# NICTA/revrand

Measured on AMD Instinct MI355X. Metric: feature-rows/sec (Phi + PhiT Phi + PhiT y) at N=10M D=32 F=4096, higher is better.
Workload: dtype f32; 1 GPU; RandomRBF nbases=2048 (F=4096), D=32, N=10000000 f32, features + MFMA Gram, rows sharded over 1 GPU(s); rows_per_gpu=10000000, device=(gfx950:sramecc+:xnack-), gram_engine=f32

## Files before the change

### revrand_amd/csrc/rr_rff.hip

```cpp
#include "rr_syrk_args.h"
#include <algorithm>
#include <map>
#include <mutex>
#include <type_traits>




__device__ __forceinline__ void sincos_rev(float t, float &s, float &c) {
    const float f = t - __builtin_rintf(t);
    s = __builtin_amdgcn_sinf(f);
    c = __builtin_amdgcn_cosf(f);
}

__device__ __forceinline__ void sincos_rev(double t, double &s, double &c) { rr_sincos_rev_f64(t, s, c); }
typedef double doublex4 __attribute__((ext_vector_type(4)));

template <int DMAX, bool GUARD, typename TX, typename TC>
__device__ __forceinline__ TC project_row(const TX *__restrict__ xr, int d, const TC (&w)[DMAX]) {
    TC z = 0;
#pragma unroll
    for (int i = 0; i < DMAX; ++i) {
        if (!GUARD || i < d) z = fma((TC)xr[i], w[i], z);
    }
// ... 829 lines not shown
#undef RR_PAIRR

__global__ void __launch_bounds__(GR_THREADS, 2)
rr_syrk_f32_ragged_kernel(const SyrkArgs p) {
    __shared__ float lds[2 * GR_KB * GR_LD];
    const int lane = threadIdx.x & 63;
    const int wave = __builtin_amdgcn_readfirstlane(threadIdx.x >> 6);
    const int last = p.nb - 1;
    const int ta = blockIdx.x % last;
    const int ks = blockIdx.x / last;
    const int ca = last * GR_TC;
    const int cb = ta * GR_TC;
    const int64_t row_begin = (int64_t)ks * p.rows_per_split;
    int64_t row_end = row_begin + p.rows_per_split;
    if (row_end > p.rows) row_end = p.rows;
    const int64_t nkb = (row_end - row_begin) / GR_KB;
    RR_DEV_ASSERT(p.rows % GR_KB == 0 && p.rows_per_split % GR_KB == 0 && p.nb * GR_TC == p.ldp && p.F > ca);
    const int w = p.F + (p.bcol ? 1 : 0) - ca;
    int ni = (w - (wave >> 2) * 128 + 31) / 32;
    ni = ni < 0 ? 0 : (ni > 4 ? 4 : ni);
    switch (ni) {
        case 0: syrk_ragged_loop<0>(p, lds, wave, lane, ca, cb, row_begin, nkb, ks); break;
        case 1: syrk_ragged_loop<1>(p, lds, wave, lane, ca, cb, row_begin, nkb, ks); break;
        case 2: syrk_ragged_loop<2>(p, lds, wave, lane, ca, cb, row_begin, nkb, ks); break;
        case 3: syrk_ragged_loop<3>(p, lds, wave, lane, ca, cb, row_begin, nkb, ks); break;
        default: syrk_ragged_loop<4>(p, lds, wave, lane, ca, cb, row_begin, nkb, ks); break;
    }
}

__constant__ unsigned char RR_DIAG_I[8][5] = {{0, 0, 0, 0, 0}, {1, 1, 1, 1, 1}, {2, 2, 2, 2, 2}, {3, 3, 3, 3, 3},
                                              {0, 0, 0, 7, 0}, {1, 1, 6, 6, 1}, {2, 5, 5, 5, 2}, {4, 4, 4, 4, 4}};
__constant__ unsigned char RR_DIAG_J[8][5] = {{0, 1, 2, 3, 4}, {1, 2, 3, 4, 5}, {2, 3, 4, 5, 6}, {3, 4, 5, 6, 7},
                                              {5, 6, 7, 7, 5}, {6, 7, 6, 7, 6}, {7, 5, 6, 7, 7}, {4, 5, 6, 7, 4}};

template <int NB>
struct KOpsD {
    float2v a[NB], b[NB];
    template <int P>
    __device__ __forceinline__ void load(const unsigned (&abase)[NB], const unsigned (&bbase)[NB]) {
#pragma unroll
        for (int e = 0; e < NB; ++e) a[e] = lds_read2st64<16 * P, 16 * P + 8>(abase[e]);
#pragma unroll
        for (int e = 0; e < NB; ++e) b[e] = lds_read2st64<16 * P, 16 * P + 8>(bbase[e]);
    }
};

template <int NB, int FIRST, int LAST>
__device__ __forceinline__ void gram_mfma_d(const KOpsD<NB> &o, floatx16 (&acc)[NB]) {
#pragma unroll
    for (int q = FIRST; q < LAST; ++q)
        acc[q % NB] = __builtin_amdgcn_mfma_f32_32x32x2f32(o.a[q % NB][q / NB], o.b[q % NB][q / NB], acc[q % NB], 0, 0, 0);
}

#define RR_PAIRD(P, CUR, NXT)                                  \
    lds_wait();                                                \
    __builtin_amdgcn_sched_barrier(0);                         \
    gram_mfma_d<NB, 0, 1>(CUR, acc);                           \
    __builtin_amdgcn_sched_barrier(0);                         \
    if ((P) + 1 < 8) NXT.template load<((P) + 1) & 7>(abase, bbase); \
    __builtin_amdgcn_sched_barrier(0);                         \
    gram_mfma_d<NB, 1, 2 * NB>(CUR, acc);                      \
    __builtin_amdgcn_sched_barrier(0);

template <int NB>
__device__ __forceinline__ void syrk_diag_body(const SyrkArgs &p, float *lds, int wave, int lane) {
    const int ta = blockIdx.x % p.nb;
    const int ks = blockIdx.x / p.nb;
    const int ca = ta * GR_TC;

    const int64_t row_begin = (int64_t)ks * p.rows_per_split;
    int64_t row_end = row_begin + p.rows_per_split;
    if (row_end > p.rows) row_end = p.rows;

    const unsigned lds0 = (unsigned)(size_t)(__attribute__((address_space(3))) float *)lds;
    const unsigned lane_off = 4u * ((lane >> 5) * GR_TC + (lane & 31));
    int bi[NB], bj[NB];
#pragma unroll
    for (int e = 0; e < NB; ++e) {
        bi[e] = RR_DIAG_I[wave][e];
        bj[e] = RR_DIAG_J[wave][e];
    }
    floatx16 acc[NB];
#pragma unroll
    for (int e = 0; e < NB; ++e)
#pragma unroll
        for (int k = 0; k < 16; ++k) acc[e][k] = 0.f;

    auto dma_tile = [&](float *buf, int64_t kb0) {
#pragma unroll
        for (int k = 0; k < 4; ++k) {
            const int lr = 4 * wave + k;
            RR_DEV_ASSERT(kb0 + lr < p.rows && ca + GR_TC <= p.ldp && p.rows % GR_KB == 0 && p.rows_per_split % GR_KB == 0);
            const float *src = p.P + (kb0 + lr) * p.ldp + ca + 4 * lane;
            __builtin_amdgcn_global_load_lds((gptr_t)src, (lptr_t)(buf + lr * GR_TC), 16, 0, 0);
        }
    };

    const int64_t nkb = (row_end - row_begin) / GR_KB;
    if (nkb > 0) {
        dma_tile(lds, row_begin);
        __syncthreads();
        for (int64_t kb = 0; kb < nkb; ++kb) {
            const int cbuf = (int)(kb & 1);
            if (kb + 1 < nkb) dma_tile(lds + (cbuf ^ 1) * (GR_KB * GR_TC), row_begin + (kb + 1) * GR_KB);
            unsigned abase[NB], bbase[NB];
#pragma unroll
            for (int e = 0; e < NB; ++e) {
                abase[e] = lds0 + cbuf * (4u * GR_KB * GR_TC) + lane_off + 128u * bi[e];
                bbase[e] = lds0 + cbuf * (4u * GR_KB * GR_TC) + lane_off + 128u * bj[e];
            }
            KOpsD<NB> o0, o1;
            o0.template load<0>(abase, bbase);
            RR_PAIRD(0, o0, o1) RR_PAIRD(1, o1, o0) RR_PAIRD(2, o0, o1) RR_PAIRD(3, o1, o0)
            RR_PAIRD(4, o0, o1) RR_PAIRD(5, o1, o0) RR_PAIRD(6, o0, o1) RR_PAIRD(7, o1, o0)
            __syncthreads();
        }
    }

    const int64_t F = p.F;
    const int hi = lane >> 5;
#pragma unroll
    for (int e = 0; e < NB; ++e) {
        const int64_t gc = ca + 32 * bj[e] + (lane & 31);
#pragma unroll
        for (int k = 0; k < 16; ++k) {
            const int64_t gr = ca + 32 * bi[e] + (k & 3) + 8 * (k >> 2) + 4 * hi;
            if (gr <= gc) rr_syrk_out(p, ks, gr, gc, acc[e][k]);
        }
    }
    (void)F;
}
#undef RR_PAIRD

__global__ void __launch_bounds__(GR_THREADS, 2)
rr_syrk_f32_diag_kernel(const SyrkArgs p) {
    __shared__ float lds[2 * GR_KB * GR_TC];
    const int lane = threadIdx.x & 63;
    const int wave = __builtin_amdgcn_readfirstlane(threadIdx.x >> 6);
    if (wave < 4)
        syrk_diag_body<5>(p, lds, wave, lane);
    else
        syrk_diag_body<4>(p, lds, wave, lane);
}

typedef float floatx4 __attribute__((ext_vector_type(4)));

template <int OFF>
__device__ __forceinline__ float lds_read_b32_off(unsigned addr) {
    float r;
    asm volatile("ds_read_b32 %0, %1 offset:%2" : "=v"(r) : "v"(addr), "i"(OFF));
    return r;
}

template <int NB, int ED>
struct KOpsD16 {
    float2v a[NB], b[NB];
    float x0, x1;
    template <int P>
    __device__ __forceinline__ void load(const unsigned (&abase)[NB], const unsigned (&bbase)[NB], unsigned xbase) {
#pragma unroll
        for (int e = 0; e < NB; ++e)
            if (e != ED) a[e] = lds_read2st64<16 * P, 16 * P + 8>(abase[e]);
#pragma unroll
        for (int e = 0; e < NB; ++e)
            if (e != ED) b[e] = lds_read2st64<16 * P, 16 * P + 8>(bbase[e]);
        x0 = lds_read_b32_off<4096 * P>(xbase);
        x1 = lds_read_b32_off<4096 * P + 64>(xbase);
    }
};

template <int NB, int ED, int FIRST, int LAST>
__device__ __forceinline__ void gram_mfma_d16(const KOpsD16<NB, ED> &o, floatx16 (&acc)[NB], floatx4 (&dd)[3]) {
#pragma unroll
    for (int q = FIRST; q < LAST; ++q) {
        if (q < NB - 1 || q >= NB + 2) {
            const int s_ = q < NB - 1 ? 0 : 1;
            const int r_ = q < NB - 1 ? q : q - (NB + 2);
            const int e = r_ < ED ? r_ : r_ + 1;
            acc[e] = __builtin_amdgcn_mfma_f32_32x32x2f32(o.a[e][s_], o.b[e][s_], acc[e], 0, 0, 0);
        } else {
            const int t = q - (NB - 1);
            dd[t] = __builtin_amdgcn_mfma_f32_16x16x4f32(t == 2 ? o.x1 : o.x0, t == 0 ? o.x0 : o.x1, dd[t], 0, 0, 0);
        }
    }
}

#define RR_PAIRD16(P, CUR, NXT)                                \
    lds_wait();                                                \
    __builtin_amdgcn_sched_barrier(0);                         \
    gram_mfma_d16<NB, ED, 0, 1>(CUR, acc, dd);                 \
    __builtin_amdgcn_sched_barrier(0);                         \
    if ((P) + 1 < KB / 4) NXT.template load<((P) + 1) & (KB / 4 - 1)>(abase, bbase, xbase); \
    __builtin_amdgcn_sched_barrier(0);                         \
    gram_mfma_d16<NB, ED, 1, 2 * NB + 1>(CUR, acc, dd);        \
    __builtin_amdgcn_sched_barrier(0);

template <int NB, int ED, int KB>
__device__ __forceinline__ void syrk_diag16_body(const SyrkArgs &p, float *lds, int wave, int lane, const unsigned bid) {
    const int ta = bid % p.nb;
    const int ks = bid / p.nb;
    const int ca = ta * GR_TC;
    const int64_t row_begin = (int64_t)ks * p.rows_per_split;
    int64_t row_end = row_begin + p.rows_per_split;
    if (row_end > p.rows) row_end = p.rows;

    const unsigned lds0 = (unsigned)(size_t)(__attribute__((address_space(3))) float *)lds;
    const unsigned lane_off = 4u * ((lane >> 5) * GR_TC + (lane & 31));
    int bi[NB], bj[NB];
#pragma unroll
    for (int e = 0; e < NB; ++e) {
        bi[e] = RR_DIAG_I[wave][e];
        bj[e] = RR_DIAG_J[wave][e];
    }
    RR_DEV_ASSERT(bi[ED] == bj[ED]);
    const unsigned lane_off16 = 4u * ((lane >> 4) * GR_TC + 32 * bi[ED] + (lane & 15));
    floatx16 acc[NB];
    floatx4 dd[3];
#pragma unroll
    for (int e = 0; e < NB; ++e)
#pragma unroll
        for (int k = 0; k < 16; ++k) acc[e][k] = 0.f;
#pragma unroll
    for (int t = 0; t < 3; ++t) dd[t] = floatx4{0.f, 0.f, 0.f, 0.f};

    const unsigned voff = 16u * lane, ldp4 = (unsigned)p.ldp * 4u;
    auto dma_tile = [&](float *buf, int64_t kb0) {
        RR_DEV_ASSERT(kb0 + KB <= p.rows && ca + GR_TC <= p.ldp && p.rows % KB == 0 && p.rows_per_split % KB == 0);
        const rr_rsrc_t ra = rr_make_rsrc(p.P + kb0 * p.ldp + ca, 0x7fffffffu);
#pragma unroll
        for (int k = 0; k < KB / 8; ++k) {
            const int lr = (KB / 8) * wave + k;
            __builtin_amdgcn_raw_ptr_buffer_load_lds(ra, (lptr_t)(buf + lr * GR_TC), 16, voff, (unsigned)lr * ldp4, 0, 0);
        }
    };

    const int64_t nkb = (row_end - row_begin) / KB;
    if (nkb > 0) {
        dma_tile(lds, row_begin);
        __syncthreads();
        for (int64_t kb = 0; kb < nkb; ++kb) {
            const int cbuf = (int)(kb & 1);
            const int slot = p.spread ? rr_dma_slot(wave, p.spread) : 0;
            auto dma_next = [&]() {
                if (kb + 1 < nkb) dma_tile(lds + (cbuf ^ 1) * (KB * GR_TC), row_begin + (kb + 1) * KB);
            };
            if (slot == 0) dma_next();
            unsigned abase[NB], bbase[NB];
#pragma unroll
            for (int e = 0; e < NB; ++e) {
                abase[e] = lds0 + cbuf * (4u * KB * GR_TC) + lane_off + 128u * bi[e];
                bbase[e] = lds0 + cbuf * (4u * KB * GR_TC) + lane_off + 128u * bj[e];
            }
            const unsigned xbase = lds0 + cbuf * (4u * KB * GR_TC) + lane_off16;
            KOpsD16<NB, ED> o0, o1;
            o0.template load<0>(abase, bbase, xbase);
            RR_PAIRD16(0, o0, o1)
            if (slot == 1) dma_next();
            RR_PAIRD16(1, o1, o0)
            if (slot == 2) dma_next();
            RR_PAIRD16(2, o0, o1)
            if (slot == 3) dma_next();
            RR_PAIRD16(3, o1, o0)
            RR_PAIRD16(4, o0, o1) RR_PAIRD16(5, o1, o0) RR_PAIRD16(6, o0, o1) RR_PAIRD16(7, o1, o0)
            if constexpr (KB == 64) {
                RR_PAIRD16(8, o0, o1) RR_PAIRD16(9, o1, o0) RR_PAIRD16(10, o0, o1) RR_PAIRD16(11, o1, o0)
                RR_PAIRD16(12, o0, o1) RR_PAIRD16(13, o1, o0) RR_PAIRD16(14, o0, o1) RR_PAIRD16(15, o1, o0)
            }
            __syncthreads();
        }
    }

    const int hi = lane >> 5;
#pragma unroll
    for (int e = 0; e < NB; ++e) {
        if (e == ED) continue;
        const int64_t gc = ca + 32 * bj[e] + (lane & 31);
#pragma unroll
        for (int k = 0; k < 16; ++k) {
            const int64_t gr = ca + 32 * bi[e] + (k & 3) + 8 * (k >> 2) + 4 * hi;
            if (gr <= gc) rr_syrk_out(p, ks, gr, gc, acc[e][k]);
        }
    }
#pragma unroll
    for (int t = 0; t < 3; ++t) {
        const int64_t gc = ca + 32 * bi[ED] + (t >= 1 ? 16 : 0) + (lane & 15);
#pragma unroll
        for (int k = 0; k < 4; ++k) {
            const int64_t gr = ca + 32 * bi[ED] + (t == 2 ? 16 : 0) + 4 * (lane >> 4) + k;
            if (gr <= gc) rr_syrk_out(p, ks, gr, gc, dd[t][k]);
        }
    }
}
#undef RR_PAIRD16

template <int KB>
__device__ __forceinline__ void syrk_diag16_dispatch(const SyrkArgs &p, float *lds, const unsigned bid) {
    const int lane = threadIdx.x & 63;
    const int wave = __builtin_amdgcn_readfirstlane(threadIdx.x >> 6);
    switch (wave) {
        case 0: case 1: case 2: case 3: syrk_diag16_body<5, 0, KB>(p, lds, wave, lane, bid); break;
        case 4: syrk_diag16_body<4, 3, KB>(p, lds, wave, lane, bid); break;
        case 5: syrk_diag16_body<4, 2, KB>(p, lds, wave, lane, bid); break;
        case 6: syrk_diag16_body<4, 1, KB>(p, lds, wave, lane, bid); break;
        default: syrk_diag16_body<4, 0, KB>(p, lds, wave, lane, bid); break;
    }
}

template <int KB>
__global__ void __launch_bounds__(GR_THREADS, 2)
rr_syrk_f32_diag16_kernel(const SyrkArgs p) {
    __shared__ float lds[2 * KB * GR_TC];
    syrk_diag16_dispatch<KB>(p, lds, blockIdx.x);
}

constexpr int GS_TC = 128, GS_KB = 32, GS_LD = 2 * GS_TC, GS_THREADS = 256;

__global__ void __launch_bounds__(GS_THREADS, 2)
rr_syrk_f32_small_kernel(const SyrkArgs p) {
    __shared__ __attribute__((aligned(16))) float lds[2][GS_KB * GS_LD];
    const int tid = threadIdx.x, lane = tid & 63, wave = tid >> 6, wr = wave >> 1, wc = wave & 1;
    const int nb = (int)(p.ldp / GS_TC);
    const int64_t ks = blockIdx.x / p.ntiles;
    int t = (int)(blockIdx.x % p.ntiles), ta = 0;
    while (t >= nb - ta) {
        t -= nb - ta;
        ++ta;
    }
    const int tb = ta + t;
    const int64_t ca = (int64_t)ta * GS_TC, cb = (int64_t)tb * GS_TC;
    const int64_t r0 = ks * p.rows_per_split;
    int64_t r1 = r0 + p.rows_per_split;
    if (r1 > p.rows) r1 = p.rows;
    const int nkb = (int)((r1 - r0 + GS_KB - 1) / GS_KB);
    floatx16 acc[2][2];
#pragma unroll
    for (int i = 0; i < 2; ++i)
#pragma unroll
        for (int j = 0; j < 2; ++j)
#pragma unroll
            for (int e = 0; e < 16; ++e) acc[i][j][e] = 0.f;
    const int lr = tid >> 5, lc = tid & 31;
    float4 ra[4], rb[4];
    auto gload = [&](int kb) {
        const float *base = p.P + (r0 + (int64_t)kb * GS_KB + lr) * p.ldp;
#pragma unroll
        for (int u = 0; u < 4; ++u) {
            ra[u] = *(const float4 *)(base + (int64_t)8 * u * p.ldp + ca + 4 * lc);
            rb[u] = *(const float4 *)(base + (int64_t)8 * u * p.ldp + cb + 4 * lc);
        }
    };
    auto lstore = [&](int buf) {
#pragma unroll
        for (int u = 0; u < 4; ++u) {
            *(float4 *)&lds[buf][(lr + 8 * u) * GS_LD + 4 * lc] = ra[u];
            *(float4 *)&lds[buf][(lr + 8 * u) * GS_LD + GS_TC + 4 * lc] = rb[u];
        }
    };
    if (nkb > 0) {
        gload(0);
        lstore(0);
    }
    __syncthreads();
    const int i32 = lane & 31, kk = lane >> 5;
    for (int kb = 0; kb < nkb; ++kb) {
        const int cur = kb & 1;
        if (kb + 1 < nkb) gload(kb + 1);
        const float *L = lds[cur];
#pragma unroll
        for (int k2 = 0; k2 < GS_KB; k2 += 2) {
            const float *row = L + (k2 + kk) * GS_LD;
            const float a0 = row[wr * 64 + i32], a1 = row[wr * 64 + 32 + i32];
            const float b0 = row[GS_TC + wc * 64 + i32], b1 = row[GS_TC + wc * 64 + 32 + i32];
            acc[0][0] = __builtin_amdgcn_mfma_f32_32x32x2f32(a0, b0, acc[0][0], 0, 0, 0);
            acc[0][1] = __builtin_amdgcn_mfma_f32_32x32x2f32(a0, b1, acc[0][1], 0, 0, 0);
            acc[1][0] = __builtin_amdgcn_mfma_f32_32x32x2f32(a1, b0, acc[1][0], 0, 0, 0);
            acc[1][1] = __builtin_amdgcn_mfma_f32_32x32x2f32(a1, b1, acc[1][1], 0, 0, 0);
        }
        if (kb + 1 < nkb) lstore(cur ^ 1);
        __syncthreads();
    }
#pragma unroll
    for (int i = 0; i < 2; ++i)
#pragma unroll
        for (int j = 0; j < 2; ++j) {
            const int64_t gc = cb + wc * 64 + 32 * j + i32;
#pragma unroll
            for (int e = 0; e < 16; ++e) {
                const int64_t gr = ca + wr * 64 + 32 * i + (e & 3) + 8 * (e >> 2) + 4 * kk;
                if (gr <= gc) rr_syrk_out(p, ks, gr, gc, acc[i][j][e]);
            }
        }
}

__global__ void __launch_bounds__(GR_THREADS, 2)
rr_syrk_f32_merged_kernel(const SyrkArgs p, const SyrkArgs pd, const unsigned n_off) {
    __shared__ float lds[2 * GR_KB * GR_LD];
    if (blockIdx.x < n_off) rr_syrk_f32_body<3>(p, lds, blockIdx.x);
    else syrk_diag16_dispatch<32>(pd, lds, blockIdx.x - n_off);
}

constexpr int G64_TC = 128;
constexpr int G64_KB = 16;
constexpr int G64_LDB = 2 * G64_TC * 8 + 128;
constexpr int G64_THREADS = 256;

struct Syrk64Args {
    const double *P;
    int64_t rows, ldp;
    int F, nb, ntiles;
    int64_t rows_per_split;
    double *G;
    int offdiag_only;
    int lower_tri = 0;
    double *part = nullptr;
    int64_t part_stride = 0;
};

__device__ __forceinline__ void rr_syrk64_out(const Syrk64Args &p, int64_t ks, int64_t gr, int64_t gc, double v) {
    if (p.part != nullptr) p.part[ks * p.part_stride + gr * p.ldp + gc] = v;
    else unsafeAtomicAdd(&p.G[gr * (int64_t)p.F + gc], v);
}

template <typename T>
__global__ void __launch_bounds__(256)
rr_syrk_det_reduce_kernel(const T *__restrict__ part, int64_t stride, int64_t ldp, int F, int nsplit, double *__restrict__ G,
                          double *__restrict__ bcol) {
    const int64_t gc = (int64_t)blockIdx.x * 256 + threadIdx.x, gr = blockIdx.y;
    if (gc < gr || gc > F || (gc == F && bcol == nullptr)) return;
    const T *q = part + gr * ldp + gc;
    double s = 0.0;
    for (int k = 0; k < nsplit; ++k) s += (double)q[(int64_t)k * stride];
    if (gc < F) G[gr * (int64_t)F + gc] += s;
    else bcol[gr] += s;
}

template <int OFF>
__device__ __forceinline__ double lds_read_b64(unsigned addr) {
    double r;
    asm volatile("ds_read_b64 %0, %1 offset:%2" : "=v"(r) : "v"(addr), "i"(OFF));
    return r;
}

struct KOps64 {
    double a[4], b[4];
    template <int T>
    __device__ __forceinline__ void load(unsigned abase, unsigned bbase) {
#pragma unroll
        for (int i = 0; i < 4; ++i) a[i] = 0;
        a[0] = lds_read_b64<4 * T * G64_LDB + 0 * 128>(abase);
        a[1] = lds_read_b64<4 * T * G64_LDB + 1 * 128>(abase);
        a[2] = lds_read_b64<4 * T * G64_LDB + 2 * 128>(abase);
        a[3] = lds_read_b64<4 * T * G64_LDB + 3 * 128>(abase);
        b[0] = lds_read_b64<4 * T * G64_LDB + 0 * 128>(bbase);
        b[1] = lds_read_b64<4 * T * G64_LDB + 1 * 128>(bbase);
        b[2] = lds_read_b64<4 * T * G64_LDB + 2 * 128>(bbase);
        b[3] = lds_read_b64<4 * T * G64_LDB + 3 * 128>(bbase);
    }
};

template <int FIRST, int LAST>
__device__ __forceinline__ void gram64_mfma(const KOps64 &o, doublex4 (&acc)[4][4]) {
#pragma unroll
    for (int q = FIRST; q < LAST; ++q)
        acc[q >> 2][q & 3] = __builtin_amdgcn_mfma_f64_16x16x4f64(o.a[q >> 2], o.b[q & 3], acc[q >> 2][q & 3], 0, 0, 0);
// ... 912 lines not shown
                const int cost = (have[ta[t]] ? 0 : 1) + ((have[tb[t]] || tb[t] == ta[t]) ? 0 : 1);
                if (cost < bestcost) { bestcost = cost; best = t; }
            }
            used[best] = 1;
            have[ta[best]] = have[tb[best]] = 1;
            part[best] = x;
        }
    }
    static const bool anneal = !(getenv("RR_GRAM_TILE_ANNEAL") && atoi(getenv("RR_GRAM_TILE_ANNEAL")) == 0);
    if (anneal && nxcd > 1 && ntiles >= 2 * nxcd && nb <= 128) {
        std::vector<int> cnt((size_t)nxcd * nb, 0);
        auto add = [&](int x, int t, int d) {
            cnt[(size_t)x * nb + ta[t]] += d;
            if (tb[t] != ta[t]) cnt[(size_t)x * nb + tb[t]] += d;
        };
        for (int t = 0; t < ntiles; ++t) add(part[t], t, 1);
        auto cost_of = [&]() {
            int c2 = 0;
            for (size_t i = 0; i < cnt.size(); ++i) c2 += cnt[i] > 0;
            return c2;
        };
        auto delta_one = [&](int x, int out, int in) {
            int before = 0, after = 0;
            const int bl[4] = {ta[out], tb[out], ta[in], tb[in]};
            for (int i = 0; i < 4; ++i) {
                bool seen = false;
                for (int j = 0; j < i; ++j) seen = seen || bl[j] == bl[i];
                if (seen) continue;
                const int b = bl[i];
                const int c0 = cnt[(size_t)x * nb + b];
                const int c1 = c0 - ((ta[out] == b) || (tb[out] == b) ? 1 : 0) + ((ta[in] == b) || (tb[in] == b) ? 1 : 0);
                before += c0 > 0;
                after += c1 > 0;
            }
            return after - before;
        };
        uint64_t rng = 0x9E3779B97F4A7C15ull;
        auto next = [&]() {
            rng ^= rng << 13; rng ^= rng >> 7; rng ^= rng << 17;
            return rng;
        };
        int cur = cost_of(), best = cur;
        std::vector<int> best_part = part;
        const int64_t iters = std::min<int64_t>((int64_t)20000 * ntiles, 6000000);
        for (int64_t it = 0; it < iters; ++it) {
            const int t1 = (int)(next() % (uint64_t)ntiles), t2 = (int)(next() % (uint64_t)ntiles);
            const int x = part[t1], y = part[t2];
            if (x == y) continue;
            const int d = delta_one(x, t1, t2) + delta_one(y, t2, t1);
            const double temp = 0.4 * (1.0 - (double)it / (double)iters) + 0.05;
            if (d <= 0 || (double)(next() >> 11) / 9007199254740992.0 < exp(-(double)d / temp)) {
                add(x, t1, -1); add(y, t2, -1); add(x, t2, 1); add(y, t1, 1);
                part[t1] = y; part[t2] = x;
                cur += d;
                if (cur < best) { best = cur; best_part = part; }
            }
        }
        part = best_part;
    }
    std::vector<int> fill(nxcd, 0);
    for (int t = 0; t < ntiles; ++t) map[(size_t)fill[part[t]]++ * nxcd + part[t]] = t;
}


int rr_launch_syrk_f32(rr_ctx *c, const float *P, int64_t rows, int64_t ldp, int F, double *dG, hipEvent_t mid,
                       double *bcol = nullptr) {
    if (c->gram_engine != 0) {
        RR_REQUIRE(bcol == nullptr, "gram: the rider column needs the f32 engine");
        RR_REQUIRE(!c->deterministic, "gram: deterministic mode (rr_set_deterministic) needs the f32 engine, not a split 16-bit one");
        return rr_launch_syrk_bf16(c, c->gram_engine, P, nullptr, rows, ldp, F, dG, mid);
    }
    RR_REQUIRE(bcol == nullptr || F < ldp, "gram: no pad column for the rider");
    static const bool small_off = getenv("RR_SYRK_SMALL") != nullptr && atoi(getenv("RR_SYRK_SMALL")) == 0;
    const int64_t big_tiles = (ldp / GR_TC) * (ldp / GR_TC + 1) / 2;
    if (!small_off && ldp <= 1024 && big_tiles * ((rows + 1023) / 1024) < c->num_cu && rows % GS_KB == 0 && !getenv("RR_GRAM_ABLATE")) {
        const int nbs = (int)(ldp / GS_TC), nt = nbs * (nbs + 1) / 2;
        int64_t ns = std::max<int64_t>((2 * c->num_cu + nt - 1) / nt, (rows + 32767) / 32768);
        ns = std::min<int64_t>(ns, std::max<int64_t>(rows / 128, 1));
        const int64_t rps_s = ((rows + ns - 1) / ns + GS_KB - 1) / GS_KB * GS_KB;
        ns = (rows + rps_s - 1) / rps_s;
        SyrkArgs a;
        a.P = P; a.rows = rows; a.ldp = ldp; a.F = F; a.nb = nbs; a.ntiles = nt; a.rows_per_split = rps_s; a.G = dG;
        a.bcol = bcol; a.tile_map = nullptr; a.offdiag_only = 0; a.ablate = 0;
        if (c->deterministic) {
            void *slabs = nullptr;
            int rc = rr_det_scratch(c, (size_t)ns * (size_t)ldp * (size_t)ldp * sizeof(float), &slabs);
            if (rc != RR_OK) return rc;
            a.part = (float *)slabs;
            a.part_stride = ldp * ldp;
        }
        hipLaunchKernelGGL(rr_syrk_f32_small_kernel, dim3((unsigned)(ns * nt)), dim3(GS_THREADS), 0, c->stream, a);
        if (mid) RR_CHECK_HIP(hipEventRecord(mid, c->stream));
        if (a.part)
            hipLaunchKernelGGL(rr_syrk_det_reduce_kernel<float>, dim3((unsigned)((F + 1 + 255) / 256), (unsigned)F), dim3(256), 0,
                               c->stream, a.part, a.part_stride, ldp, F, (int)ns, dG, bcol);
        RR_CHECK_HIP(hipGetLastError());
        return RR_OK;
    }
    const int nb_all = (int)(ldp / GR_TC);
    const int od = (nb_all >= 2 && !getenv("RR_SYRK_NO_DIAG_KERNEL")) ? 1 : 0;
    const int w_last = F + (bcol ? 1 : 0) - GR_TC * (nb_all - 1);
    const int rg = (od && nb_all >= 3 && w_last <= 192 && !getenv("RR_SYRK_NO_RAGGED_KERNEL")) ? 1 : 0;
    const int nb = nb_all - rg;
    const int ntiles = od ? nb * (nb - 1) / 2 : nb * (nb + 1) / 2;
    const int nxcd = 8;
    const bool use_map = (ntiles % nxcd == 0) && !getenv("RR_GRAM_NO_TILE_MAP");
    if (use_map && c->tile_map_nb != nb * 2 + od) {
        std::vector<int> map;
        rr_build_tile_map(nb, od, nxcd, map);
        if (c->tile_map) (void)hipFree(c->tile_map);
        c->tile_map = nullptr;
        RR_CHECK_HIP(hipMalloc((void **)&c->tile_map, map.size() * sizeof(int)));
        RR_CHECK_HIP(hipMemcpy(c->tile_map, map.data(), map.size() * sizeof(int), hipMemcpyHostToDevice));
        c->tile_map_nb = nb * 2 + od;
    }
    const int64_t total_tiles = (int64_t)nb_all * (nb_all + 1) / 2;
    auto gcd64 = [](int64_t x, int64_t y) { while (y) { const int64_t u = x % y; x = y; y = u; } return x; };
    const int64_t min_splits = (rows + 32767) / 32768;
    auto rows_per = [&](int64_t ns) { return ((rows + ns - 1) / ns + GR_KB - 1) / GR_KB * GR_KB; };
    const int64_t unit = ntiles > 0 ? c->num_cu / gcd64(c->num_cu, ntiles) : 1;
    int64_t nsplit = (min_splits + unit - 1) / unit * unit;
    auto floor_rows = [&](int64_t tiles_per_split) {
        return tiles_per_split * ((rows + 1023) / 1024) < c->num_cu ? (int64_t)256 : (int64_t)1024;
    };
    auto small_split = [&](int64_t tiles_per_split) {
        const int64_t fr = floor_rows(tiles_per_split);
        if (fr == 1024) return (rows + 1023) / 1024;
        const int64_t want = (c->num_cu + tiles_per_split - 1) / std::max<int64_t>(tiles_per_split, 1);
        return std::min((rows + fr - 1) / fr, std::max((rows + 1023) / 1024, want));
    };
    if (rows / nsplit < 1024) {
        nsplit = small_split(std::max(ntiles, 1));
        static const bool no_search = getenv("RR_SYRK_SPLIT_SEARCH") != nullptr && atoi(getenv("RR_SYRK_SPLIT_SEARCH")) == 0;
        if (ntiles > 0 && !no_search) {
            double best_cost = 1e300;
            int64_t best_ns = nsplit;
            const int64_t ns_hi = std::max<int64_t>(rows / 256, 1), ns_lo = std::max<int64_t>(rows / 32768, 1);
            for (int64_t ns = ns_lo; ns <= ns_hi && ns <= ns_lo + 4096; ++ns) {
                const int64_t rp = rows_per(ns), n2 = (rows + rp - 1) / rp;
                const int64_t rounds = ((int64_t)ntiles * n2 + c->num_cu - 1) / c->num_cu;
                const double cost = (double)rounds * ((double)rp + 96.0);
                if (cost < best_cost - 1e-9) {
                    best_cost = cost;
                    best_ns = n2;
                }
            }
            nsplit = best_ns;
        }
    }
    if (nsplit < 1) nsplit = 1;
    int64_t rps = rows_per(nsplit);
    int64_t nsplit_d = nsplit, rps_d = rps;
    if (od) {
        double best = -1.0;
        for (int64_t ns = min_splits; ns < min_splits + 96; ++ns) {
            if (rows / ns < floor_rows(nb_all) && ns > 1) break;
            const int64_t wg = ns * nb_all, rounds = (wg + c->num_cu - 1) / c->num_cu;
            const double eff = (double)wg / (double)(rounds * c->num_cu);
            if (eff > best + 1e-9) {
                best = eff;
                nsplit_d = ns;
            }
        }
        rps_d = rows_per(nsplit_d);
        if (rows % 64 == 0 && getenv("RR_SYRK_DIAG_KB") != nullptr && atoi(getenv("RR_SYRK_DIAG_KB")) == 64)
            rps_d = (rps_d + 63) / 64 * 64;
    }
    int64_t nsplit_r = nsplit, rps_r = rps;
    if (rg) {
        double best = -1.0;
        for (int64_t ns = min_splits; ns < min_splits + 96; ++ns) {
            if (rows / ns < floor_rows(nb_all - 1) && ns > 1) break;
            const int64_t wg = ns * (nb_all - 1), rounds = (wg + c->num_cu - 1) / c->num_cu;
            const double eff = (double)wg / (double)(rounds * c->num_cu);
            if (eff > best + 1e-9) {
                best = eff;
                nsplit_r = ns;
            }
        }
        rps_r = rows_per(nsplit_r);
    }
    const char *renv = getenv("RR_GRAM_ROWS_PER_SPLIT");
    if (renv && atoll(renv) >= GR_KB) rps = rps_d = rps_r = (atoll(renv) / GR_KB) * GR_KB;
    if (c->deterministic) rps_d = rps_r = rps;
    nsplit = (rows + rps - 1) / rps;
    nsplit_d = (rows + rps_d - 1) / rps_d;
    nsplit_r = (rows + rps_r - 1) / rps_r;
    RR_REQUIRE(nsplit * total_tiles < (int64_t)1 << 31 && nsplit_d * nb_all < (int64_t)1 << 31 &&
                   nsplit_r * nb_all < (int64_t)1 << 31, "gram: grid too large");
    SyrkArgs a;
    a.P = P; a.rows = rows; a.ldp = ldp; a.F = F; a.nb = nb; a.ntiles = ntiles; a.rows_per_split = rps; a.G = dG;
    a.bcol = bcol;
    a.tile_map = use_map ? c->tile_map : nullptr;
    a.offdiag_only = od;
    a.ablate = getenv("RR_GRAM_ABLATE") ? atoi(getenv("RR_GRAM_ABLATE")) : 0;
    a.spread = rr_dma_spread_env();
    if (c->deterministic) {
        void *slabs = nullptr;
        int rc = rr_det_scratch(c, (size_t)nsplit * (size_t)ldp * (size_t)ldp * sizeof(float), &slabs);
        if (rc != RR_OK) return rc;
        a.part = (float *)slabs;
        a.part_stride = ldp * ldp;
    }
    static const int syrk_mode = getenv("RR_SYRK_STAGGER") ? atoi(getenv("RR_SYRK_STAGGER")) : 3;
    static const bool merge_diag = getenv("RR_SYRK_MERGE_DIAG") != nullptr && atoi(getenv("RR_SYRK_MERGE_DIAG")) != 0;
    if (merge_diag && od && !rg && ntiles > 0 && syrk_mode == 3 && !a.ablate && !getenv("RR_SYRK_NO_DIAG16")) {
        SyrkArgs ad = a;
        ad.nb = nb_all;
        ad.rows_per_split = rps_d;
        const unsigned n_off = (unsigned)(nsplit * ntiles);
        hipLaunchKernelGGL(rr_syrk_f32_merged_kernel, dim3(n_off + (unsigned)(nsplit_d * nb_all)), dim3(GR_THREADS), 0, c->stream, a, ad, n_off);
        if (mid) RR_CHECK_HIP(hipEventRecord(mid, c->stream));
        if (a.part)
            hipLaunchKernelGGL(rr_syrk_det_reduce_kernel<float>, dim3((unsigned)((F + 1 + 255) / 256), (unsigned)F), dim3(256), 0,
                               c->stream, a.part, a.part_stride, ldp, F, (int)nsplit, dG, bcol);
        RR_CHECK_HIP(hipGetLastError());
        return RR_OK;
    }
    if (ntiles > 0) {
        if (syrk_mode == 1 && !a.ablate)
            hipLaunchKernelGGL(rr_syrk_f32_flatstag_kernel, dim3((unsigned)(nsplit * ntiles)), dim3(GR_THREADS), 0, c->stream, a);
        else if (syrk_mode == 2 && !a.ablate)
            hipLaunchKernelGGL(rr_syrk_f32_buf_kernel, dim3((unsigned)(nsplit * ntiles)), dim3(GR_THREADS), 0, c->stream, a);
        else if (syrk_mode == 0 || a.ablate)
            hipLaunchKernelGGL(rr_syrk_f32_flat_kernel, dim3((unsigned)(nsplit * ntiles)), dim3(GR_THREADS), 0, c->stream, a);
        else
            hipLaunchKernelGGL(rr_syrk_f32_kernel, dim3((unsigned)(nsplit * ntiles)), dim3(GR_THREADS), 0, c->stream, a);
    }
    if (rg) {
        SyrkArgs ar = a;
        ar.nb = nb_all;
        ar.rows_per_split = rps_r;
        hipLaunchKernelGGL(rr_syrk_f32_ragged_kernel, dim3((unsigned)(nsplit_r * (nb_all - 1))), dim3(GR_THREADS), 0, c->stream, ar);
    }
    if (mid) RR_CHECK_HIP(hipEventRecord(mid, c->stream));
    if (od) {
        SyrkArgs ad = a;
        ad.nb = nb_all;
        ad.rows_per_split = rps_d;
        static const bool no_diag16 = getenv("RR_SYRK_NO_DIAG16") != nullptr;
        static const bool kb64 = getenv("RR_SYRK_DIAG_KB") != nullptr && atoi(getenv("RR_SYRK_DIAG_KB")) == 64;
        if (no_diag16)
            hipLaunchKernelGGL(rr_syrk_f32_diag_kernel, dim3((unsigned)(nsplit_d * nb_all)), dim3(GR_THREADS), 0, c->stream, ad);
        else if (kb64 && rows % 64 == 0 && ad.rows_per_split % 64 == 0)
            hipLaunchKernelGGL(rr_syrk_f32_diag16_kernel<64>, dim3((unsigned)(nsplit_d * nb_all)), dim3(GR_THREADS), 0, c->stream, ad);
        else
            hipLaunchKernelGGL(rr_syrk_f32_diag16_kernel<32>, dim3((unsigned)(nsplit_d * nb_all)), dim3(GR_THREADS), 0, c->stream, ad);
    }
    if (a.part)
        hipLaunchKernelGGL(rr_syrk_det_reduce_kernel<float>, dim3((unsigned)((F + 1 + 255) / 256), (unsigned)F), dim3(256), 0,
                           c->stream, a.part, a.part_stride, ldp, F, (int)nsplit, dG, bcol);
    RR_CHECK_HIP(hipGetLastError());
    return RR_OK;
}

int rr_launch_syrk_f64(rr_ctx *c, const double *P, int64_t rows, int64_t ldp, int F, double *dG, int lower_tri = 0) {
    const int nb = (int)(ldp / G64_TC);
    const int od = (nb >= 2 && !getenv("RR_SYRK_NO_DIAG_KERNEL")) ? 1 : 0;
    const int ntiles = od ? nb * (nb - 1) / 2 : nb * (nb + 1) / 2;
    const int64_t slots = (int64_t)c->num_cu * 2;
    int64_t g = slots, t = ntiles;
    while (t) { const int64_t u = g % t; g = t; t = u; }
    const int64_t unit = slots / g;
    static const bool no_fine = getenv("RR_SYRK64_FINE_SPLIT") != nullptr && atoi(getenv("RR_SYRK64_FINE_SPLIT")) == 0;
    const int64_t min_rows = (lower_tri && rows == ldp && rows <= 2048 && !no_fine) ? 128 : 512;
    int64_t nsplit = unit;
    if (rows / nsplit < 2048) nsplit = (slots * 4 + ntiles - 1) / ntiles;
    if (rows / nsplit < min_rows) nsplit = (rows + min_rows - 1) / min_rows;
    if (nsplit < 1) nsplit = 1;
    const int64_t rps = ((rows + nsplit - 1) / nsplit + G64_KB - 1) / G64_KB * G64_KB;
    nsplit = (rows + rps - 1) / rps;
    RR_REQUIRE(nsplit * ntiles < (int64_t)1 << 31, "gram: grid too large");
    Syrk64Args a;
    a.P = P; a.rows = rows; a.ldp = ldp; a.F = F; a.nb = nb; a.ntiles = ntiles; a.rows_per_split = rps; a.G = dG;
    a.offdiag_only = od;
    static const bool no_tri = getenv("RR_SYRK64_TRI") != nullptr && atoi(getenv("RR_SYRK64_TRI")) == 0;
    a.lower_tri = lower_tri && !no_tri && rows == ldp ? 1 : 0;
    if (c->deterministic) {
        void *slabs = nullptr;
        int rc = rr_det_scratch(c, (size_t)nsplit * (size_t)ldp * (size_t)ldp * sizeof(double), &slabs);
        if (rc != RR_OK) return rc;
        a.part = (double *)slabs;
        a.part_stride = ldp * ldp;
    }
    if (ntiles > 0)
        hipLaunchKernelGGL(rr_syrk_f64_kernel, dim3((unsigned)(nsplit * ntiles)), dim3(G64_THREADS), 0, c->stream, a);
    if (od) {
        const int64_t dslots = (int64_t)c->num_cu * 4;
        int64_t best_ns = 1;
        double best = -1.0;
        for (int64_t ns = 1; ns <= 4 * dslots / nb + 1; ++ns) {
            if (rows / ns < min_rows && ns > 1) break;
            const int64_t wg = ns * nb, rounds = (wg + dslots - 1) / dslots;
            const double eff = (double)wg / (double)(rounds * dslots);
            if (eff > best + 1e-9) {
                best = eff;
                best_ns = ns;
            }
        }
        Syrk64Args ad = a;
        ad.rows_per_split = ((rows + best_ns - 1) / best_ns + G64_KB - 1) / G64_KB * G64_KB;
        if (c->deterministic) ad.rows_per_split = rps;
        const int64_t nsd = (rows + ad.rows_per_split - 1) / ad.rows_per_split;
        hipLaunchKernelGGL(rr_syrk_f64_diag_kernel, dim3((unsigned)(nsd * nb)), dim3(G64_THREADS), 0, c->stream, ad);
    }
    if (a.part)
        hipLaunchKernelGGL(rr_syrk_det_reduce_kernel<double>, dim3((unsigned)((F + 255) / 256), (unsigned)F), dim3(256), 0,
                           c->stream, a.part, a.part_stride, ldp, F, (int)nsplit, dG, (double *)nullptr);
    RR_CHECK_HIP(hipGetLastError());
    return RR_OK;
}
// ... 877 lines not shown
```

Measured before the change: 8.457 million feature-rows/s.

## Redeal diagonal-tile Gram work across waves and size splits by occupancy

Reassigns the 32x32 sub-blocks of each diagonal Gram tile to the eight waves through a new operand-deal table. Each wave now loads a small set of shared column operands and forms several off-diagonal and diagonal products from them, so fewer LDS reads are needed per MFMA and the work per wave is more even. Diagonal blocks are computed with 16x16 MFMAs per wave role. Separately, the host split heuristic for the diagonal kernel now counts occupancy slots (workgroups per CU) instead of CU count when choosing the number of row splits. The changes add template complexity and change register pressure per role.

```diff
diff --git a/revrand_amd/csrc/rr_rff.hip b/revrand_amd/csrc/rr_rff.hip
--- a/revrand_amd/csrc/rr_rff.hip
+++ b/revrand_amd/csrc/rr_rff.hip
@@ -1005,35 +1005,62 @@
     return r;
 }
 
-template <int NB, int ED>
+__constant__ unsigned char RR_DEAL_OP[8][4] = {{0, 1, 4, 5}, {0, 1, 6, 7}, {2, 3, 4, 5}, {2, 3, 6, 7},
+                                               {0, 1, 2, 3}, {1, 2, 3, 3}, {4, 5, 6, 7}, {5, 6, 7, 7}};
+
+template <int ROLE>
+struct DiagDeal;
+template <>
+struct DiagDeal<0> {
+    static constexpr int NO = 4, NB = 4, ND = 0;
+    __host__ __device__ static constexpr int ia(int e) { return e >> 1; }
+    __host__ __device__ static constexpr int ib(int e) { return 2 + (e & 1); }
+    __host__ __device__ static constexpr int dg(int) { return 0; }
+};
+template <>
+struct DiagDeal<1> {
+    static constexpr int NO = 4, NB = 3, ND = 2;
+    __host__ __device__ static constexpr int ia(int) { return 0; }
+    __host__ __device__ static constexpr int ib(int e) { return e + 1; }
+    __host__ __device__ static constexpr int dg(int d) { return d; }
+};
+template <>
+struct DiagDeal<2> {
+    static constexpr int NO = 3, NB = 3, ND = 2;
+    __host__ __device__ static constexpr int ia(int e) { return e >> 1; }
+    __host__ __device__ static constexpr int ib(int e) { return e == 0 ? 1 : 2; }
+    __host__ __device__ static constexpr int dg(int d) { return d + 1; }
+};
+
+template <class D>
 struct KOpsD16 {
-    float2v a[NB], b[NB];
-    float x0, x1;
+    static constexpr int NX = D::ND > 0 ? D::ND : 1;
+    float2v o[D::NO];
+    float x0[NX], x1[NX];
     template <int P>
-    __device__ __forceinline__ void load(const unsigned (&abase)[NB], const unsigned (&bbase)[NB], unsigned xbase) {
-#pragma unroll
-        for (int e = 0; e < NB; ++e)
-            if (e != ED) a[e] = lds_read2st64<16 * P, 16 * P + 8>(abase[e]);
-#pragma unroll
-        for (int e = 0; e < NB; ++e)
-            if (e != ED) b[e] = lds_read2st64<16 * P, 16 * P + 8>(bbase[e]);
-        x0 = lds_read_b32_off<4096 * P>(xbase);
-        x1 = lds_read_b32_off<4096 * P + 64>(xbase);
+    __device__ __forceinline__ void load(const unsigned (&obase)[D::NO], const unsigned (&xbase)[NX]) {
+#pragma unroll
+        for (int i = 0; i < D::NO; ++i) o[i] = lds_read2st64<16 * P, 16 * P + 8>(obase[i]);
+#pragma unroll
+        for (int d = 0; d < D::ND; ++d) {
+            x0[d] = lds_read_b32_off<4096 * P>(xbase[d]);
+            x1[d] = lds_read_b32_off<4096 * P + 64>(xbase[d]);
+        }
     }
 };
 
-template <int NB, int ED, int FIRST, int LAST>
-__device__ __forceinline__ void gram_mfma_d16(const KOpsD16<NB, ED> &o, floatx16 (&acc)[NB], floatx4 (&dd)[3]) {
+template <class D, int FIRST, int LAST>
+__device__ __forceinline__ void gram_mfma_d16(const KOpsD16<D> &o, floatx16 (&acc)[D::NB], floatx4 (&dd)[3 * KOpsD16<D>::NX]) {
+    constexpr int NB = D::NB, ND = D::ND;
 #pragma unroll
     for (int q = FIRST; q < LAST; ++q) {
-        if (q < NB - 1 || q >= NB + 2) {
-            const int s_ = q < NB - 1 ? 0 : 1;
-            const int r_ = q < NB - 1 ? q : q - (NB + 2);
-            const int e = r_ < ED ? r_ : r_ + 1;
-            acc[e] = __builtin_amdgcn_mfma_f32_32x32x2f32(o.a[e][s_], o.b[e][s_], acc[e], 0, 0, 0);
+        if (q < NB || q >= NB + 3 * ND) {
+            const int s_ = q < NB ? 0 : 1;
+            const int e = q < NB ? q : q - (NB + 3 * ND);
+            acc[e] = __builtin_amdgcn_mfma_f32_32x32x2f32(o.o[D::ia(e)][s_], o.o[D::ib(e)][s_], acc[e], 0, 0, 0);
         } else {
-            const int t = q - (NB - 1);
-            dd[t] = __builtin_amdgcn_mfma_f32_16x16x4f32(t == 2 ? o.x1 : o.x0, t == 0 ? o.x0 : o.x1, dd[t], 0, 0, 0);
+            const int d = (q - NB) / 3, t = (q - NB) % 3;
+            dd[3 * d + t] = __builtin_amdgcn_mfma_f32_16x16x4f32(t == 2 ? o.x1[d] : o.x0[d], t == 0 ? o.x0[d] : o.x1[d], dd[3 * d + t], 0, 0, 0);
         }
     }
 }
@@ -1041,15 +1068,17 @@
 #define RR_PAIRD16(P, CUR, NXT)                                \
     lds_wait();                                                \
     __builtin_amdgcn_sched_barrier(0);                         \
-    gram_mfma_d16<NB, ED, 0, 1>(CUR, acc, dd);                 \
+    gram_mfma_d16<D, 0, 1>(CUR, acc, dd);                      \
     __builtin_amdgcn_sched_barrier(0);                         \
-    if ((P) + 1 < KB / 4) NXT.template load<((P) + 1) & (KB / 4 - 1)>(abase, bbase, xbase); \
+    if ((P) + 1 < KB / 4) NXT.template load<((P) + 1) & (KB / 4 - 1)>(obase, xbase); \
     __builtin_amdgcn_sched_barrier(0);                         \
-    gram_mfma_d16<NB, ED, 1, 2 * NB + 1>(CUR, acc, dd);        \
+    gram_mfma_d16<D, 1, 2 * D::NB + 3 * D::ND>(CUR, acc, dd);  \
     __builtin_amdgcn_sched_barrier(0);
 
-template <int NB, int ED, int KB>
+template <int ROLE, int KB>
 __device__ __forceinline__ void syrk_diag16_body(const SyrkArgs &p, float *lds, int wave, int lane, const unsigned bid) {
+    using D = DiagDeal<ROLE>;
+    constexpr int NO = D::NO, NB = D::NB, ND = D::ND, NX = KOpsD16<D>::NX;
     const int ta = bid % p.nb;
     const int ks = bid / p.nb;
     const int ca = ta * GR_TC;
@@ -1059,22 +1088,19 @@
 
     const unsigned lds0 = (unsigned)(size_t)(__attribute__((address_space(3))) float *)lds;
     const unsigned lane_off = 4u * ((lane >> 5) * GR_TC + (lane & 31));
-    int bi[NB], bj[NB];
-#pragma unroll
-    for (int e = 0; e < NB; ++e) {
-        bi[e] = RR_DIAG_I[wave][e];
-        bj[e] = RR_DIAG_J[wave][e];
-    }
-    RR_DEV_ASSERT(bi[ED] == bj[ED]);
-    const unsigned lane_off16 = 4u * ((lane >> 4) * GR_TC + 32 * bi[ED] + (lane & 15));
+    const unsigned lane_off16 = 4u * ((lane >> 4) * GR_TC + (lane & 15));
+    int op[NO];
+#pragma unroll
+    for (int i = 0; i < NO; ++i) op[i] = RR_DEAL_OP[wave][i];
+    RR_DEV_ASSERT(op[NO - 1] < 8 && op[D::ia(NB - 1)] < op[D::ib(NB - 1)]);
     floatx16 acc[NB];
-    floatx4 dd[3];
+    floatx4 dd[3 * NX];
 #pragma unroll
     for (int e = 0; e < NB; ++e)
 #pragma unroll
         for (int k = 0; k < 16; ++k) acc[e][k] = 0.f;
 #pragma unroll
-    for (int t = 0; t < 3; ++t) dd[t] = floatx4{0.f, 0.f, 0.f, 0.f};
+    for (int t = 0; t < 3 * NX; ++t) dd[t] = floatx4{0.f, 0.f, 0.f, 0.f};
 
     const unsigned voff = 16u * lane, ldp4 = (unsigned)p.ldp * 4u;
     auto dma_tile = [&](float *buf, int64_t kb0) {
@@ -1098,15 +1124,13 @@
                 if (kb + 1 < nkb) dma_tile(lds + (cbuf ^ 1) * (KB * GR_TC), row_begin + (kb + 1) * KB);
             };
             if (slot == 0) dma_next();
-            unsigned abase[NB], bbase[NB];
-#pragma unroll
-            for (int e = 0; e < NB; ++e) {
-                abase[e] = lds0 + cbuf * (4u * KB * GR_TC) + lane_off + 128u * bi[e];
-                bbase[e] = lds0 + cbuf * (4u * KB * GR_TC) + lane_off + 128u * bj[e];
-            }
-            const unsigned xbase = lds0 + cbuf * (4u * KB * GR_TC) + lane_off16;
-            KOpsD16<NB, ED> o0, o1;
-            o0.template load<0>(abase, bbase, xbase);
+            unsigned obase[NO], xbase[NX];
+#pragma unroll
+            for (int i = 0; i < NO; ++i) obase[i] = lds0 + cbuf * (4u * KB * GR_TC) + lane_off + 128u * op[i];
+#pragma unroll
+            for (int d = 0; d < NX; ++d) xbase[d] = lds0 + cbuf * (4u * KB * GR_TC) + lane_off16 + 128u * op[D::dg(d)];
+            KOpsD16<D> o0, o1;
+            o0.template load<0>(obase, xbase);
             RR_PAIRD16(0, o0, o1)
             if (slot == 1) dma_next();
             RR_PAIRD16(1, o1, o0)
@@ -1126,21 +1150,24 @@
     const int hi = lane >> 5;
 #pragma unroll
     for (int e = 0; e < NB; ++e) {
-        if (e == ED) continue;
-        const int64_t gc = ca + 32 * bj[e] + (lane & 31);
+        const int64_t gc = ca + 32 * op[D::ib(e)] + (lane & 31);
 #pragma unroll
         for (int k = 0; k < 16; ++k) {
-            const int64_t gr = ca + 32 * bi[e] + (k & 3) + 8 * (k >> 2) + 4 * hi;
+            const int64_t gr = ca + 32 * op[D::ia(e)] + (k & 3) + 8 * (k >> 2) + 4 * hi;
             if (gr <= gc) rr_syrk_out(p, ks, gr, gc, acc[e][k]);
         }
     }
 #pragma unroll
-    for (int t = 0; t < 3; ++t) {
-        const int64_t gc = ca + 32 * bi[ED] + (t >= 1 ? 16 : 0) + (lane & 15);
-#pragma unroll
-        for (int k = 0; k < 4; ++k) {
-            const int64_t gr = ca + 32 * bi[ED] + (t == 2 ? 16 : 0) + 4 * (lane >> 4) + k;
-            if (gr <= gc) rr_syrk_out(p, ks, gr, gc, dd[t][k]);
+    for (int d = 0; d < ND; ++d) {
+        const int64_t c0 = ca + 32 * op[D::dg(d)];
+#pragma unroll
+        for (int t = 0; t < 3; ++t) {
+            const int64_t gc = c0 + (t >= 1 ? 16 : 0) + (lane & 15);
+#pragma unroll
+            for (int k = 0; k < 4; ++k) {
+                const int64_t gr = c0 + (t == 2 ? 16 : 0) + 4 * (lane >> 4) + k;
+                if (gr <= gc) rr_syrk_out(p, ks, gr, gc, dd[3 * d + t][k]);
+            }
         }
     }
 }
@@ -1151,18 +1178,19 @@
     const int lane = threadIdx.x & 63;
     const int wave = __builtin_amdgcn_readfirstlane(threadIdx.x >> 6);
     switch (wave) {
-        case 0: case 1: case 2: case 3: syrk_diag16_body<5, 0, KB>(p, lds, wave, lane, bid); break;
-        case 4: syrk_diag16_body<4, 3, KB>(p, lds, wave, lane, bid); break;
-        case 5: syrk_diag16_body<4, 2, KB>(p, lds, wave, lane, bid); break;
-        case 6: syrk_diag16_body<4, 1, KB>(p, lds, wave, lane, bid); break;
-        default: syrk_diag16_body<4, 0, KB>(p, lds, wave, lane, bid); break;
-    }
-}
-
+        case 0: case 1: case 2: case 3: syrk_diag16_body<0, KB>(p, lds, wave, lane, bid); break;
+        case 4: case 6: syrk_diag16_body<1, KB>(p, lds, wave, lane, bid); break;
+        default: syrk_diag16_body<2, KB>(p, lds, wave, lane, bid); break;
+    }
+}
+
+#ifndef RR_DIAG16_LDS_PAD
+#define RR_DIAG16_LDS_PAD 0
+#endif
 template <int KB>
 __global__ void __launch_bounds__(GR_THREADS, 2)
 rr_syrk_f32_diag16_kernel(const SyrkArgs p) {
-    __shared__ float lds[2 * KB * GR_TC];
+    __shared__ float lds[2 * KB * GR_TC + (KB == 32 ? RR_DIAG16_LDS_PAD : 0)];
     syrk_diag16_dispatch<KB>(p, lds, blockIdx.x);
 }
 
@@ -2381,11 +2409,19 @@
     int64_t rps = rows_per(nsplit);
     int64_t nsplit_d = nsplit, rps_d = rps;
     if (od) {
+        static const int diag_wg_per_cu = [] {
+            int n = 1;
+            if (hipOccupancyMaxActiveBlocksPerMultiprocessor(&n, rr_syrk_f32_diag16_kernel<32>, GR_THREADS, 0) != hipSuccess) n = 1;
+            const char *e = getenv("RR_SYRK_DIAG_KB");
+            if (getenv("RR_SYRK_NO_DIAG16") || getenv("RR_SYRK_MERGE_DIAG") || (e && atoi(e) == 64)) n = 1;
+            return n >= 2 ? 2 : 1;
+        }();
+        const int64_t slots = (int64_t)c->num_cu * diag_wg_per_cu;
         double best = -1.0;
         for (int64_t ns = min_splits; ns < min_splits + 96; ++ns) {
             if (rows / ns < floor_rows(nb_all) && ns > 1) break;
-            const int64_t wg = ns * nb_all, rounds = (wg + c->num_cu - 1) / c->num_cu;
-            const double eff = (double)wg / (double)(rounds * c->num_cu);
+            const int64_t wg = ns * nb_all, rounds = (wg + slots - 1) / slots;
+            const double eff = (double)wg / (double)(rounds * slots);
             if (eff > best + 1e-9) {
                 best = eff;
                 nsplit_d = ns;
```

After: 8.472 million feature-rows/s, median of 5. About the same (+0.2%).
